# impromptuRong/hd_yolo

Hardware: NVIDIA B200
Metric: postproc_tiles_per_s (higher is better)
Workload: dtype f32

## Files before the change

hd_yolo_b200/csrc/merge.cu:

```cuda
#include "hdy_common.cuh"

namespace hdy {

enum : uint8_t { MS_UNKNOWN = 0, MS_KEPT = 1, MS_SUPPRESSED = 2, MS_DROPPED = 3, MS_REMOTE_UNKNOWN = 4 };

constexpr int kMergeThreads = 256;
constexpr int kMaxRounds = 64;
constexpr float kMergeCellMargin = 1.01f;
constexpr float kMergeMaxScaled = 1.0e6f;

constexpr int kExtBins = 128;
struct MergeStats {
  float ext_sum;
  unsigned ext_cnt;
  float cell_size;
  unsigned ext_hist[kExtBins];
  int unknown[kMaxRounds + 1];
  int rounds_run;
};

constexpr int kScanThreads = 1024;
constexpr int kScanItems = 4;
constexpr int kScanTile = kScanThreads * kScanItems;

__device__ __forceinline__ int block_scan_1024(int v, int* warp_tmp, int& total) {
  const int lane = threadIdx.x & 31, warp = threadIdx.x >> 5;
  int incl = v;
#pragma unroll
  for (int o = 1; o < 32; o <<= 1) {
    int u = __shfl_up_sync(0xffffffffu, incl, o);
    if (lane >= o) incl += u;
  }
  if (lane == 31) warp_tmp[warp] = incl;
  __syncthreads();
  if (warp == 0) {
    int s = warp_tmp[lane], t = s;
#pragma unroll
    for (int o = 1; o < 32; o <<= 1) {
      int u = __shfl_up_sync(0xffffffffu, t, o);
      if (lane >= o) t += u;
    }
    warp_tmp[lane] = t - s;
    if (lane == 31) warp_tmp[32] = t;
  }
  __syncthreads();
  const int excl = warp_tmp[warp] + incl - v;
  total = warp_tmp[32];
  __syncthreads();
  return excl;
}

__global__ void __launch_bounds__(kScanThreads) scan_reduce_kernel(const int* __restrict__ a, long long n,
                                                                    int* __restrict__ block_sums) {
  __shared__ int warp_tmp[33];
  const long long base = (long long)blockIdx.x * kScanTile + (long long)threadIdx.x * kScanItems;
  int s = 0;
#pragma unroll
  for (int k = 0; k < kScanItems; ++k)
    if (base + k < n) s += a[base + k];
  int total;
  block_scan_1024(s, warp_tmp, total);
  if (threadIdx.x == 0) block_sums[blockIdx.x] = total;
}

__global__ void __launch_bounds__(kScanThreads) scan_sums_kernel(int* __restrict__ block_sums, int nblocks,
                                                                  int* __restrict__ total_out) {
  __shared__ int warp_tmp[33];
  __shared__ int carry;
  if (threadIdx.x == 0) carry = 0;
  __syncthreads();
  for (int b0 = 0; b0 < nblocks; b0 += kScanThreads) {
    const int i = b0 + threadIdx.x;
    const int v = i < nblocks ? block_sums[i] : 0;
    int total;
    const int excl = block_scan_1024(v, warp_tmp, total);
    if (i < nblocks) block_sums[i] = carry + excl;
    __syncthreads();
    if (threadIdx.x == 0) carry += total;
    __syncthreads();
  }
  if (threadIdx.x == 0 && total_out) *total_out = carry;
}

__global__ void __launch_bounds__(kScanThreads) scan_apply_kernel(int* __restrict__ a, long long n,
                                                                   const int* __restrict__ block_sums) {
  __shared__ int warp_tmp[33];
  const long long base = (long long)blockIdx.x * kScanTile + (long long)threadIdx.x * kScanItems;
  int v[kScanItems], s = 0;
#pragma unroll
  for (int k = 0; k < kScanItems; ++k) {
    v[k] = (base + k < n) ? a[base + k] : 0;
    s += v[k];
  }
  int total;
  int run = block_sums[blockIdx.x] + block_scan_1024(s, warp_tmp, total);
#pragma unroll
  for (int k = 0; k < kScanItems; ++k) {
    if (base + k < n) a[base + k] = run;
    run += v[k];
  }
}

static inline size_t scan_scratch_ints(long long n) { return (size_t)((n + kScanTile - 1) / kScanTile) + 1; }

static int device_exclusive_scan(int* a, long long n, int* scratch, int* total_out, cudaStream_t st) {
  if (n <= 0) return HDY_OK;
  const int nblocks = (int)((n + kScanTile - 1) / kScanTile);
  scan_reduce_kernel<<<nblocks, kScanThreads, 0, st>>>(a, n, scratch);
  scan_sums_kernel<<<1, kScanThreads, 0, st>>>(scratch, nblocks, total_out);
  scan_apply_kernel<<<nblocks, kScanThreads, 0, st>>>(a, n, scratch);
  return check_launch("device_exclusive_scan");
}

__global__ void __launch_bounds__(1024) append_offsets_kernel(const int32_t* __restrict__ counts, int bs,
                                                               long long* __restrict__ cursor,
                                                               long long* __restrict__ tile_offsets) {
  __shared__ int warp_tmp[33];
  __shared__ long long carry;
  if (threadIdx.x == 0) carry = *cursor;
  __syncthreads();
  for (int b0 = 0; b0 < bs; b0 += 1024) {
    const int i = b0 + threadIdx.x;
    const int v = i < bs ? max(counts[i], 0) : 0;
    int total;
    const int excl = block_scan_1024(v, warp_tmp, total);
    if (i < bs) tile_offsets[i] = carry + excl;
    __syncthreads();
    if (threadIdx.x == 0) carry += total;
    __syncthreads();
  }
  if (threadIdx.x == 0) {
    tile_offsets[bs] = carry;
    *cursor = carry;
  }
}

__global__ void append_tiles_kernel(const float4* __restrict__ boxes, const float* __restrict__ scores,
                                    const int64_t* __restrict__ labels, const uint8_t* __restrict__ fragile,
                                    const int32_t* __restrict__ counts,
                                    const float4* __restrict__ rois, int max_det, int tile_base, float scale,
                                    const long long* __restrict__ tile_offsets, long long capacity,
                                    float4* __restrict__ out_boxes, float* __restrict__ out_scores,
                                    int64_t* __restrict__ out_labels, int32_t* __restrict__ out_tile,
                                    int32_t* __restrict__ status) {
  const int tile = blockIdx.y;
  const int k = min(max(counts[tile], 0), max_det);
  const long long off = tile_offsets[tile];
  const float4 roi = rois[tile];
  for (int d = blockIdx.x * blockDim.x + threadIdx.x; d < k; d += gridDim.x * blockDim.x) {
    const long long o = off + d;
    if (o >= capacity) {
      atomicOr(status, HDY_STATUS_OVERFLOW);
      continue;
    }
    const size_t s = (size_t)tile * max_det + d;
    float4 b = boxes[s];
    if (scale != 1.0f) {
      b.x = __fmul_rn(b.x, scale);
// ... 492 lines not shown
constexpr int kSelMaxBlocks = 4096;

__global__ void __launch_bounds__(kSelThreads) select_count_kernel(const uint8_t* __restrict__ state,
                                                                   const long long* __restrict__ n_dev,
                                                                   long long n_max, long long chunk,
                                                                   int* __restrict__ block_counts) {
  const long long n = n_dev ? min(*n_dev, n_max) : n_max;
  const long long lo = (long long)blockIdx.x * chunk, hi = min(lo + chunk, n);
  int c = 0;
  for (long long i = lo + threadIdx.x; i < hi; i += kSelThreads) c += state[i] == MS_KEPT;
  __shared__ int part[kSelThreads / 32];
#pragma unroll
  for (int o = 16; o > 0; o >>= 1) c += __shfl_xor_sync(0xffffffffu, c, o);
  if ((threadIdx.x & 31) == 0) part[threadIdx.x >> 5] = c;
  __syncthreads();
  if (threadIdx.x == 0) {
    int t = 0;
    for (int w = 0; w < kSelThreads / 32; ++w) t += part[w];
    block_counts[blockIdx.x] = t;
  }
}

__global__ void __launch_bounds__(1024) select_scan_kernel(int* __restrict__ block_counts, int nblocks,
                                                           int* __restrict__ count_out) {
  __shared__ int warp_tmp[33];
  int v[4], s = 0;
#pragma unroll
  for (int j = 0; j < 4; ++j) {
    const int i = threadIdx.x * 4 + j;
    v[j] = i < nblocks ? block_counts[i] : 0;
    s += v[j];
  }
  int total;
  int excl = block_scan_1024(s, warp_tmp, total);
#pragma unroll
  for (int j = 0; j < 4; ++j) {
    const int i = threadIdx.x * 4 + j;
    if (i < nblocks) block_counts[i] = excl;
    excl += v[j];
  }
  if (threadIdx.x == 0) *count_out = total;
}

__global__ void __launch_bounds__(kSelThreads) select_write_kernel(const uint8_t* __restrict__ state,
                                                                   const float* __restrict__ scores,
                                                                   const long long* __restrict__ n_dev,
                                                                   long long n_max, long long chunk,
                                                                   const int* __restrict__ block_offsets,
                                                                   uint64_t* __restrict__ keys) {
  __shared__ int wcount[kSelThreads / 32];
  const long long n = n_dev ? min(*n_dev, n_max) : n_max;
  const long long lo = (long long)blockIdx.x * chunk, hi = min(lo + chunk, n);
  const int lane = threadIdx.x & 31, warp = threadIdx.x >> 5;
  long long running = block_offsets[blockIdx.x];
  for (long long i0 = lo; i0 < hi; i0 += kSelThreads) {
    const long long i = i0 + threadIdx.x;
    const bool k = i < hi && state[i] == MS_KEPT;
    const unsigned m = __ballot_sync(0xffffffffu, k);
    if (lane == 0) wcount[warp] = __popc(m);
    __syncthreads();
    int before = 0, total = 0;
#pragma unroll
    for (int w = 0; w < kSelThreads / 32; ++w) {
      const int c = wcount[w];
      if (w < warp) before += c;
      total += c;
    }
    if (k) keys[running + before + __popc(m & ((1u << lane) - 1u))] = make_key(scores[i], (uint32_t)i);
    running += total;
    __syncthreads();
  }
}

constexpr int kSortThreads = 256;
constexpr int kSortPerWarp = 1024;
constexpr int kSortWarps = kSortThreads / 32;

__global__ void __launch_bounds__(kSortThreads) sort_hist_kernel(const uint64_t* __restrict__ keys,
                                                                  const int* __restrict__ n_dev, int n_max, int shift,
                                                                  int n_sub, int* __restrict__ hist) {
  __shared__ int h[kSortWarps][256];
  const int n = n_dev ? min(*n_dev, n_max) : n_max;
  const int warp = threadIdx.x >> 5, lane = threadIdx.x & 31;
  const int sub = blockIdx.x * kSortWarps + warp;
  for (int d = lane; d < 256; d += 32) h[warp][d] = 0;
  __syncwarp();
  const long long b = (long long)sub * kSortPerWarp;
  for (int k = lane; k < kSortPerWarp; k += 32)
    if (b + k < n) atomicAdd(&h[warp][(int)((keys[b + k] >> shift) & 255)], 1);
  __syncwarp();
  if (sub < n_sub)
    for (int d = lane; d < 256; d += 32) hist[(size_t)d * n_sub + sub] = h[warp][d];
}

__global__ void __launch_bounds__(kSortThreads) sort_scatter_kernel(const uint64_t* __restrict__ keys,
                                                                     const int* __restrict__ n_dev, int n_max,
                                                                     int shift, int n_sub, const int* __restrict__ hist,
                                                                     uint64_t* __restrict__ out) {
  __shared__ int base[kSortWarps][256];
  const int n = n_dev ? min(*n_dev, n_max) : n_max;
  const int warp = threadIdx.x >> 5, lane = threadIdx.x & 31;
  const int sub = blockIdx.x * kSortWarps + warp;
  if (sub >= n_sub) return;
  for (int d = lane; d < 256; d += 32) base[warp][d] = hist[(size_t)d * n_sub + sub];
  __syncwarp();
  const long long b = (long long)sub * kSortPerWarp;
  for (int k0 = 0; k0 < kSortPerWarp; k0 += 32) {
    const long long i = b + k0 + lane;
    const bool valid = i < n;
    const uint64_t key = valid ? keys[i] : 0;
    const int d = valid ? (int)((key >> shift) & 255) : 256 + lane;
    const unsigned peers = __match_any_sync(0xffffffffu, d);
    const int rank = __popc(peers & ((1u << lane) - 1u));
    int dst = 0;
    if (valid) dst = base[warp][d] + rank;
    __syncwarp();
    if (valid && rank == 0) base[warp][d] += __popc(peers);
    __syncwarp();
    if (valid) out[dst] = key;
  }
}

__global__ void merge_gather_kernel(const uint64_t* __restrict__ keys, const int* __restrict__ count, int max_det,
                                    const float4* __restrict__ boxes, const float* __restrict__ scores,
                                    const int64_t* __restrict__ labels, int64_t* __restrict__ out_idx,
                                    float4* __restrict__ out_boxes, float* __restrict__ out_scores,
                                    int64_t* __restrict__ out_labels, int* __restrict__ out_count) {
  const int k = min(*count, max_det);
  if (blockIdx.x == 0 && threadIdx.x == 0) *out_count = k;
  for (int j = blockIdx.x * blockDim.x + threadIdx.x; j < k; j += gridDim.x * blockDim.x) {
    const uint32_t i = key_index(keys[j]);
    if (out_idx) out_idx[j] = (int64_t)i;
    if (out_boxes) out_boxes[j] = boxes[i];
    if (out_scores) out_scores[j] = scores[i];
    if (out_labels && labels) out_labels[j] = labels[i];
  }
}

static inline unsigned blocks_for(long long n, int threads, int max_blocks = 148 * 16) {
  long long b = (n + threads - 1) / threads;
  if (b < 1) b = 1;
  if (b > max_blocks) b = max_blocks;
  return (unsigned)b;
}

constexpr int kSeamHdr = HDY_SEAM_HDR_WORDS, kSeamFar = HDY_SEAM_FAR_WORDS, kSeamRow = HDY_SEAM_ROW_WORDS;
constexpr int kSeamMaxWorld = HDY_SEAM_MAX_WORLD;
enum { SM_NTOTAL = 0, SM_MARGIN = 2, SM_GBASE = 3, SM_FLAGS = 4, SM_FAR_TOTAL = 5, SM_UNDECIDED = 8, SM_REP_OFF = 16,
       SM_OWN_SEAM = 88 };

__device__ __forceinline__ void atomic_min_float(float* addr, float v) {
  if (v >= 0.f)
    atomicMin(reinterpret_cast<int*>(addr), __float_as_int(v));
  else
    atomicMax(reinterpret_cast<unsigned*>(addr), __float_as_uint(v));
}
__device__ __forceinline__ void atomic_max_float(float* addr, float v) {
  if (v >= 0.f)
    atomicMax(reinterpret_cast<int*>(addr), __float_as_int(v));
  else
    atomicMin(reinterpret_cast<unsigned*>(addr), __float_as_uint(v));
}

__global__ void seam_summary_pack_kernel(long long n_local, const float* __restrict__ margin,
                                         const float4* __restrict__ far_boxes, const int32_t* __restrict__ far_tile,
                                         const int32_t* __restrict__ far_count, int far_list_capacity, int tile_base,
                                         int far_cap, int32_t* __restrict__ block) {
  const int k = blockIdx.x * blockDim.x + threadIdx.x;
  const int nf = far_count ? *far_count : 0;
  if (k == 0) {
    float* f = reinterpret_cast<float*>(block);
    const float big = 3.0e38f;
    f[0] = big, f[1] = big, f[2] = -big, f[3] = -big;
    f[4] = margin ? *margin : 0.f;
    block[5] = nf > far_list_capacity ? far_cap + 1 : nf;
    *reinterpret_cast<long long*>(block + 6) = n_local;
// ... 500 lines not shown
  merge_finish_kernel<<<blocks_for(n_max, 256), 256, 0, (cudaStream_t)stream>>>(
      w.pos, w.cstate, reinterpret_cast<const long long*>(n_dev), n_max, state, status);
  return check_launch("hdy_merge_finish");
}

int hdy_merge_nms(const float* boxes, const float* scores, const int32_t* tile_id, const float* tile_cores,
                  const uint8_t* tile_dirty, const float* margin, const int64_t* n_dev, int64_t n_max, float conf_thres,
                  float iou_thres,
                  int max_rounds, uint8_t* state, int32_t* status, void* workspace, size_t workspace_bytes,
                  hdy_stream_t stream) {
  HDY_REQUIRE(max_rounds >= 1 && max_rounds <= kMaxRounds, "hdy_merge_nms: max_rounds out of range [1,%d]", kMaxRounds);
  MergeIn in;
  in.boxes = reinterpret_cast<const float4*>(boxes);
  in.scores = scores;
  in.rep_gidx = nullptr;
  in.gidx_base_dev = nullptr;
  in.tile_base = 0;
  in.tile_id = tile_id;
  in.tile_cores = reinterpret_cast<const float4*>(tile_cores);
  in.tile_dirty = tile_dirty;
  in.margin = margin;
  in.n_dev = reinterpret_cast<const long long*>(n_dev);
  in.n_max = n_max;
  in.n_local = n_max;
  in.conf = conf_thres;
  in.thr = iou_thres;
  int rc = merge_build_common("hdy_merge_nms", in, tile_cores, state, workspace, workspace_bytes, (cudaStream_t)stream);
  if (rc) return rc;
  rc = hdy_merge_rounds(workspace, n_max, iou_thres, 0, max_rounds, stream);
  if (rc) return rc;
  return hdy_merge_finish(workspace, n_dev, n_max, state, status, stream);
}

size_t hdy_sort_workspace_bytes(int64_t n_max) {
  if (n_max <= 0) return 256;
  const long long n_sub = (n_max + kSortPerWarp - 1) / kSortPerWarp;
  const long long hist = 256 * n_sub;
  return align256((size_t)hist * 4) + align256(scan_scratch_ints(hist) * 4);
}

int hdy_sort_keys_bytes(uint64_t* keys, uint64_t* tmp, const int32_t* n_dev, int64_t n_max, int first_byte,
                        int n_bytes, void* workspace, size_t workspace_bytes, hdy_stream_t stream) {
  HDY_REQUIRE(first_byte >= 0 && n_bytes >= 0 && first_byte + n_bytes <= 8 && (n_bytes & 1) == 0,
              "hdy_sort_keys_bytes: bytes [%d, %d) -- an even number of bytes inside the key", first_byte,
              first_byte + n_bytes);
  HDY_REQUIRE(n_max >= 0 && n_max < (1ll << 31), "hdy_sort_keys_bytes: bad size");
  if (n_max == 0) return HDY_OK;
  HDY_REQUIRE(keys && tmp && workspace && workspace_bytes >= hdy_sort_workspace_bytes(n_max),
              "hdy_sort_keys_bytes: NULL pointer or workspace too small");
  cudaStream_t st = (cudaStream_t)stream;
  const int n_sub = (int)((n_max + kSortPerWarp - 1) / kSortPerWarp);
  const long long hist_n = 256ll * n_sub;
  int* hist = static_cast<int*>(workspace);
  int* scratch = reinterpret_cast<int*>(static_cast<unsigned char*>(workspace) + align256((size_t)hist_n * 4));
  const unsigned blocks = (unsigned)((n_sub + kSortWarps - 1) / kSortWarps);
  uint64_t* src = keys;
  uint64_t* dst = tmp;
  for (int pass = first_byte; pass < first_byte + n_bytes; ++pass) {
    sort_hist_kernel<<<blocks, kSortThreads, 0, st>>>(src, n_dev, (int)n_max, pass * 8, n_sub, hist);
    int rc = device_exclusive_scan(hist, hist_n, scratch, nullptr, st);
    if (rc) return rc;
    sort_scatter_kernel<<<blocks, kSortThreads, 0, st>>>(src, n_dev, (int)n_max, pass * 8, n_sub, hist, dst);
    uint64_t* t = src;
    src = dst;
    dst = t;
  }
  return check_launch("hdy_sort_keys_bytes");
}

int hdy_merge_select_ordered(const uint8_t* state, const float* scores, const int64_t* n_dev, int64_t n_max,
                             uint64_t* keys, int32_t* count, int32_t* block_scratch, hdy_stream_t stream) {
  HDY_REQUIRE(n_max >= 0 && n_max < (1ll << 31) && count && block_scratch, "hdy_merge_select_ordered: bad arguments");
  cudaStream_t st = (cudaStream_t)stream;
  if (n_max == 0) {
    cudaError_t e = cudaMemsetAsync(count, 0, 4, st);
    if (e != cudaSuccess) {
      set_error("hdy_merge_select_ordered: %s", cudaGetErrorString(e));
      return HDY_ERR_CUDA;
    }
    return HDY_OK;
  }
  HDY_REQUIRE(state && scores && keys, "hdy_merge_select_ordered: NULL pointer");
  long long chunk = (n_max + kSelMaxBlocks - 1) / kSelMaxBlocks;
  chunk = ((chunk + kSelThreads - 1) / kSelThreads) * kSelThreads;
  if (chunk < 4 * kSelThreads) chunk = 4 * kSelThreads;
  const int nblocks = (int)((n_max + chunk - 1) / chunk);
  const long long* nd = reinterpret_cast<const long long*>(n_dev);
  select_count_kernel<<<nblocks, kSelThreads, 0, st>>>(state, nd, n_max, chunk, block_scratch);
  select_scan_kernel<<<1, 1024, 0, st>>>(block_scratch, nblocks, count);
  select_write_kernel<<<nblocks, kSelThreads, 0, st>>>(state, scores, nd, n_max, chunk, block_scratch, keys);
  return check_launch("hdy_merge_select_ordered");
}

int hdy_merge_gather(const uint64_t* keys, const int32_t* count, int64_t max_det, const float* boxes,
                     const float* scores, const int64_t* labels, int64_t* out_idx, float* out_boxes,
                     float* out_scores, int64_t* out_labels, int32_t* out_count, hdy_stream_t stream) {
  HDY_REQUIRE(max_det >= 0 && max_det < (1ll << 31) && keys && count && out_count, "hdy_merge_gather: bad arguments");
  HDY_REQUIRE((!out_boxes || boxes) && (!out_scores || scores), "hdy_merge_gather: output without its source");
  HDY_REQUIRE((((uintptr_t)boxes | (uintptr_t)out_boxes) & 15) == 0, "hdy_merge_gather: box arrays must be 16-byte aligned");
  merge_gather_kernel<<<blocks_for(max_det > 0 ? max_det : 1, 256), 256, 0, (cudaStream_t)stream>>>(
      keys, count, (int)max_det, reinterpret_cast<const float4*>(boxes), scores, labels, out_idx,
      reinterpret_cast<float4*>(out_boxes), out_scores, out_labels, out_count);
  return check_launch("hdy_merge_gather");
}

}
```

hd_yolo_b200/slide.py:

```python
from __future__ import annotations

import ctypes as C
from typing import Dict, List, Optional, Sequence, Tuple

import torch

from . import _lib
from ._lib import HdyError, ptr
from .ops import DetectBatch, _Scratch, _aligned16, _call, _conf_thr_f32, _iou_thr_f32, _need_cuda, _stream

__all__ = ["sliding_window_scanner", "tile_cores", "merge_outputs", "rescale_outputs", "scale_coords", "clip_coords",
           "merge_nms", "ensemble_merge", "Ensemble", "SlideAccumulator", "sort_keys", "kept_digest", "fold_digest",
           "mask_digest",
           "STATE_KEPT", "STATE_SUPPRESSED", "STATE_DROPPED"]

STATE_UNKNOWN, STATE_KEPT, STATE_SUPPRESSED, STATE_DROPPED = 0, 1, 2, 3
AFFINE_UNPAD, AFFINE_SCALE, AFFINE_CLIP, AFFINE_ROUND = 1, 2, 4, 8
_ws = _Scratch()


def _pair(v):
    return (v, v) if isinstance(v, (int, float)) else (v[0], v[1])


# ... 86 lines not shown
    while True:
        _call("hdy_merge_nms", ptr(boxes), ptr(scores), ptr(tile_id) if use_cores else None,
              ptr(cores) if use_cores else None, ptr(dirty) if use_cores else None,
              ptr(margin) if use_cores else None, ptr(n_dev), n,
              _conf_thr_f32(conf_thres), _iou_thr_f32(iou_thres), rounds, ptr(state), ptr(status), ptr(ws), wbytes,
              _stream(), launches=8 + 3 * rounds)
        if not int(status.item()) & _lib.HDY_STATUS_ROUNDS:
            return state
        if rounds >= 64:
            raise HdyError("merge NMS did not converge in 64 rounds")
        rounds, _ = min(64, rounds * 2), status.zero_()


def dirty_tiles(far_boxes: torch.Tensor, far_tile: torch.Tensor, far_count: torch.Tensor,
                rois: torch.Tensor) -> torch.Tensor:
    n_tiles = int(rois.shape[0])
    dirty = torch.empty((max(n_tiles, 1),), dtype=torch.uint8, device=rois.device)
    _call("hdy_merge_dirty_tiles", ptr(far_boxes), ptr(far_tile), ptr(far_count), int(far_boxes.shape[0]),
          ptr(_aligned16(rois.contiguous())), n_tiles, ptr(dirty), _stream())
    return dirty


def sort_keys(keys: torch.Tensor, n_dev: Optional[torch.Tensor] = None, first_byte: int = 0,
              n_bytes: int = 8) -> torch.Tensor:
    if not keys.is_cuda or keys.dtype != torch.int64 or not keys.is_contiguous():
        raise HdyError("keys must be a contiguous CUDA int64 tensor")
    n = keys.numel()
    if n:
        lib = _lib.load()
        wbytes = lib.hdy_sort_workspace_bytes(n)
        ws = _ws.get(keys.device, "sort", wbytes)
        tmp = _ws.get(keys.device, "sort_tmp", n * 8)
        _call("hdy_sort_keys_bytes", ptr(keys), ptr(tmp), ptr(n_dev), n, int(first_byte), int(n_bytes), ptr(ws), wbytes,
              _stream(), launches=int(n_bytes) * 5)
    return keys


def _order_keys(state, scores, n: int, count: torch.Tensor) -> torch.Tensor:
    dev = scores.device
    keys = torch.empty((max(n, 1),), dtype=torch.int64, device=dev)
    if n == 0:
        count.zero_()
        return keys
    blk = _ws.get(dev, "select_blocks", 4096 * 4)
    _call("hdy_merge_select_ordered", ptr(state), ptr(scores), None, n, ptr(keys), ptr(count), ptr(blk), _stream(),
          launches=3)
    sort_keys(keys, n_dev=count, first_byte=4, n_bytes=4)
    return keys


def _gather_ordered(keys, count, k_all: int, max_det: int, boxes, scores, labels):
    dev = boxes.device
    k = min(int(k_all), int(max_det))
    idx = torch.empty((k,), dtype=torch.int64, device=dev)
    ob = torch.empty((k, 4), dtype=torch.float32, device=dev)
    os_ = torch.empty((k,), dtype=torch.float32, device=dev)
    ol = torch.empty((k,), dtype=torch.int64, device=dev) if labels is not None else None
    oc = torch.empty((1,), dtype=torch.int32, device=dev)
    if k:
        _call("hdy_merge_gather", ptr(keys), ptr(count), k, ptr(boxes), ptr(scores), ptr(labels), ptr(idx), ptr(ob),
              ptr(os_), ptr(ol), ptr(oc), _stream())
    return idx, ob, os_, ol


def _kept_in_order(state, boxes, scores, labels, max_det: int, n_dev=None):
    n = boxes.shape[0]
    count = torch.empty((1,), dtype=torch.int32, device=boxes.device)
# ... 268 lines not shown
```

Before: 161,400.

## Replace per-pass histogram/scan/scatter radix sort with onesweep decoupled-lookback sort

Replaces the three-kernel-per-byte LSD radix sort (warp histograms, device-wide exclusive scan, scatter) with one upfront histogram kernel covering all digit passes, followed by a single onesweep kernel per pass. That kernel ranks keys in shared memory and resolves global offsets through a decoupled lookback over tile prefixes. This cuts the kernel launch count and per-pass global histogram traffic for the kept-box ordering sort, at the cost of spin-waiting on lookback flags and reliance on tile-ticket ordering. The gather kernel is also restructured to handle four items per thread and reuses the score stored in the key where it can.

After: 164,300 (median of 6 runs). +1.8%, better.

```diff
diff --git a/hd_yolo_b200/csrc/merge.cu b/hd_yolo_b200/csrc/merge.cu
--- a/hd_yolo_b200/csrc/merge.cu
+++ b/hd_yolo_b200/csrc/merge.cu
@@ -722,68 +722,49 @@
   }
 }
 
-constexpr int kSortThreads = 256;
-constexpr int kSortPerWarp = 1024;
-constexpr int kSortWarps = kSortThreads / 32;
-
-__global__ void __launch_bounds__(kSortThreads) sort_hist_kernel(const uint64_t* __restrict__ keys,
-                                                                  const int* __restrict__ n_dev, int n_max, int shift,
-                                                                  int n_sub, int* __restrict__ hist) {
-  __shared__ int h[kSortWarps][256];
-  const int n = n_dev ? min(*n_dev, n_max) : n_max;
-  const int warp = threadIdx.x >> 5, lane = threadIdx.x & 31;
-  const int sub = blockIdx.x * kSortWarps + warp;
-  for (int d = lane; d < 256; d += 32) h[warp][d] = 0;
-  __syncwarp();
-  const long long b = (long long)sub * kSortPerWarp;
-  for (int k = lane; k < kSortPerWarp; k += 32)
-    if (b + k < n) atomicAdd(&h[warp][(int)((keys[b + k] >> shift) & 255)], 1);
-  __syncwarp();
-  if (sub < n_sub)
-    for (int d = lane; d < 256; d += 32) hist[(size_t)d * n_sub + sub] = h[warp][d];
-}
-
-__global__ void __launch_bounds__(kSortThreads) sort_scatter_kernel(const uint64_t* __restrict__ keys,
-                                                                     const int* __restrict__ n_dev, int n_max,
-                                                                     int shift, int n_sub, const int* __restrict__ hist,
-                                                                     uint64_t* __restrict__ out) {
-  __shared__ int base[kSortWarps][256];
-  const int n = n_dev ? min(*n_dev, n_max) : n_max;
-  const int warp = threadIdx.x >> 5, lane = threadIdx.x & 31;
-  const int sub = blockIdx.x * kSortWarps + warp;
-  if (sub >= n_sub) return;
-  for (int d = lane; d < 256; d += 32) base[warp][d] = hist[(size_t)d * n_sub + sub];
-  __syncwarp();
-  const long long b = (long long)sub * kSortPerWarp;
-  for (int k0 = 0; k0 < kSortPerWarp; k0 += 32) {
-    const long long i = b + k0 + lane;
-    const bool valid = i < n;
-    const uint64_t key = valid ? keys[i] : 0;
-    const int d = valid ? (int)((key >> shift) & 255) : 256 + lane;
-    const unsigned peers = __match_any_sync(0xffffffffu, d);
-    const int rank = __popc(peers & ((1u << lane) - 1u));
-    int dst = 0;
-    if (valid) dst = base[warp][d] + rank;
-    __syncwarp();
-    if (valid && rank == 0) base[warp][d] += __popc(peers);
-    __syncwarp();
-    if (valid) out[dst] = key;
-  }
-}
-
-__global__ void merge_gather_kernel(const uint64_t* __restrict__ keys, const int* __restrict__ count, int max_det,
-                                    const float4* __restrict__ boxes, const float* __restrict__ scores,
-                                    const int64_t* __restrict__ labels, int64_t* __restrict__ out_idx,
-                                    float4* __restrict__ out_boxes, float* __restrict__ out_scores,
-                                    int64_t* __restrict__ out_labels, int* __restrict__ out_count) {
+constexpr int kGatherThreads = 256;
+constexpr int kGatherItems = 4;
+
+__global__ void __launch_bounds__(kGatherThreads) merge_gather_kernel(
+    const uint64_t* __restrict__ keys, const int* __restrict__ count, int max_det, const float4* __restrict__ boxes,
+    const float* __restrict__ scores, const int64_t* __restrict__ labels, int64_t* __restrict__ out_idx,
+    float4* __restrict__ out_boxes, float* __restrict__ out_scores, int64_t* __restrict__ out_labels,
+    int* __restrict__ out_count) {
   const int k = min(*count, max_det);
   if (blockIdx.x == 0 && threadIdx.x == 0) *out_count = k;
-  for (int j = blockIdx.x * blockDim.x + threadIdx.x; j < k; j += gridDim.x * blockDim.x) {
-    const uint32_t i = key_index(keys[j]);
-    if (out_idx) out_idx[j] = (int64_t)i;
-    if (out_boxes) out_boxes[j] = boxes[i];
-    if (out_scores) out_scores[j] = scores[i];
-    if (out_labels && labels) out_labels[j] = labels[i];
+  const bool want_labels = out_labels && labels;
+  const long long step = (long long)gridDim.x * kGatherThreads * kGatherItems;
+  for (long long j0 = (long long)blockIdx.x * kGatherThreads * kGatherItems + threadIdx.x; j0 < k; j0 += step) {
+    uint32_t row[kGatherItems];
+    float sc[kGatherItems];
+#pragma unroll
+    for (int e = 0; e < kGatherItems; ++e) {
+      const long long j = j0 + e * kGatherThreads;
+      const uint64_t key = j < k ? keys[j] : 0ull;
+      row[e] = key_index(key);
+      sc[e] = key_score(key);
+    }
+    float4 b[kGatherItems];
+    int64_t l[kGatherItems];
+#pragma unroll
+    for (int e = 0; e < kGatherItems; ++e) {
+      if (j0 + e * kGatherThreads < k) {
+        const uint32_t i = row[e];
+        if (out_boxes) b[e] = boxes[i];
+        if (want_labels) l[e] = labels[i];
+        if (out_scores && sc[e] == 0.0f) sc[e] = scores[i];
+      }
+    }
+#pragma unroll
+    for (int e = 0; e < kGatherItems; ++e) {
+      const long long j = j0 + e * kGatherThreads;
+      if (j < k) {
+        if (out_idx) out_idx[j] = (int64_t)row[e];
+        if (out_boxes) out_boxes[j] = b[e];
+        if (out_scores) out_scores[j] = sc[e];
+        if (want_labels) out_labels[j] = l[e];
+      }
+    }
   }
 }
 
@@ -1358,42 +1339,6 @@
   return hdy_merge_finish(workspace, n_dev, n_max, state, status, stream);
 }
 
-size_t hdy_sort_workspace_bytes(int64_t n_max) {
-  if (n_max <= 0) return 256;
-  const long long n_sub = (n_max + kSortPerWarp - 1) / kSortPerWarp;
-  const long long hist = 256 * n_sub;
-  return align256((size_t)hist * 4) + align256(scan_scratch_ints(hist) * 4);
-}
-
-int hdy_sort_keys_bytes(uint64_t* keys, uint64_t* tmp, const int32_t* n_dev, int64_t n_max, int first_byte,
-                        int n_bytes, void* workspace, size_t workspace_bytes, hdy_stream_t stream) {
-  HDY_REQUIRE(first_byte >= 0 && n_bytes >= 0 && first_byte + n_bytes <= 8 && (n_bytes & 1) == 0,
-              "hdy_sort_keys_bytes: bytes [%d, %d) -- an even number of bytes inside the key", first_byte,
-              first_byte + n_bytes);
-  HDY_REQUIRE(n_max >= 0 && n_max < (1ll << 31), "hdy_sort_keys_bytes: bad size");
-  if (n_max == 0) return HDY_OK;
-  HDY_REQUIRE(keys && tmp && workspace && workspace_bytes >= hdy_sort_workspace_bytes(n_max),
-              "hdy_sort_keys_bytes: NULL pointer or workspace too small");
-  cudaStream_t st = (cudaStream_t)stream;
-  const int n_sub = (int)((n_max + kSortPerWarp - 1) / kSortPerWarp);
-  const long long hist_n = 256ll * n_sub;
-  int* hist = static_cast<int*>(workspace);
-  int* scratch = reinterpret_cast<int*>(static_cast<unsigned char*>(workspace) + align256((size_t)hist_n * 4));
-  const unsigned blocks = (unsigned)((n_sub + kSortWarps - 1) / kSortWarps);
-  uint64_t* src = keys;
-  uint64_t* dst = tmp;
-  for (int pass = first_byte; pass < first_byte + n_bytes; ++pass) {
-    sort_hist_kernel<<<blocks, kSortThreads, 0, st>>>(src, n_dev, (int)n_max, pass * 8, n_sub, hist);
-    int rc = device_exclusive_scan(hist, hist_n, scratch, nullptr, st);
-    if (rc) return rc;
-    sort_scatter_kernel<<<blocks, kSortThreads, 0, st>>>(src, n_dev, (int)n_max, pass * 8, n_sub, hist, dst);
-    uint64_t* t = src;
-    src = dst;
-    dst = t;
-  }
-  return check_launch("hdy_sort_keys_bytes");
-}
-
 int hdy_merge_select_ordered(const uint8_t* state, const float* scores, const int64_t* n_dev, int64_t n_max,
                              uint64_t* keys, int32_t* count, int32_t* block_scratch, hdy_stream_t stream) {
   HDY_REQUIRE(n_max >= 0 && n_max < (1ll << 31) && count && block_scratch, "hdy_merge_select_ordered: bad arguments");
@@ -1424,7 +1369,8 @@
   HDY_REQUIRE(max_det >= 0 && max_det < (1ll << 31) && keys && count && out_count, "hdy_merge_gather: bad arguments");
   HDY_REQUIRE((!out_boxes || boxes) && (!out_scores || scores), "hdy_merge_gather: output without its source");
   HDY_REQUIRE((((uintptr_t)boxes | (uintptr_t)out_boxes) & 15) == 0, "hdy_merge_gather: box arrays must be 16-byte aligned");
-  merge_gather_kernel<<<blocks_for(max_det > 0 ? max_det : 1, 256), 256, 0, (cudaStream_t)stream>>>(
+  merge_gather_kernel<<<blocks_for(max_det > 0 ? max_det : 1, kGatherThreads * kGatherItems), kGatherThreads, 0,
+                        (cudaStream_t)stream>>>(
       keys, count, (int)max_det, reinterpret_cast<const float4*>(boxes), scores, labels, out_idx,
       reinterpret_cast<float4*>(out_boxes), out_scores, out_labels, out_count);
   return check_launch("hdy_merge_gather");
diff --git a/hd_yolo_b200/csrc/sort.cu b/hd_yolo_b200/csrc/sort.cu
--- /dev/null
+++ b/hd_yolo_b200/csrc/sort.cu
@@ -0,0 +1,257 @@
+#include "hdy_common.cuh"
+
+namespace hdy {
+
+constexpr int kSortThreads = 256;
+constexpr int kSortWarps = kSortThreads / 32;
+constexpr int kSortItems = 16;
+constexpr int kWarpKeys = kSortItems * 32;
+constexpr int kTile = kSortThreads * kSortItems;
+constexpr int kMaxDigits = 8;
+constexpr int kLookback = 16;
+
+constexpr int kHistItems = 8;
+constexpr int kHistMaxBlocks = 148 * 8;
+
+static inline size_t align256(size_t v) { return (v + 255) & ~(size_t)255; }
+
+constexpr size_t kHeadBytes = 256 * kMaxDigits * 4 + 256;
+
+__device__ __forceinline__ unsigned lanemask_lt() {
+  unsigned m;
+  asm("mov.u32 %0, %%lanemask_lt;" : "=r"(m));
+  return m;
+}
+
+__device__ __forceinline__ unsigned long long ld_relaxed(const unsigned long long* p) {
+  unsigned long long v;
+  asm volatile("ld.relaxed.gpu.global.u64 %0, [%1];" : "=l"(v) : "l"(p) : "memory");
+  return v;
+}
+
+__device__ __forceinline__ void st_relaxed(unsigned long long* p, unsigned long long v) {
+  asm volatile("st.relaxed.gpu.global.u64 [%0], %1;" ::"l"(p), "l"(v) : "memory");
+}
+
+__device__ __forceinline__ unsigned digit_peers(int d, bool valid) {
+  unsigned peers = __ballot_sync(0xffffffffu, valid);
+#pragma unroll
+  for (int bit = 0; bit < 8; ++bit) {
+    const unsigned m = __ballot_sync(0xffffffffu, (d >> bit) & 1);
+    peers &= ((d >> bit) & 1) ? m : ~m;
+  }
+  return peers;
+}
+
+__device__ __forceinline__ int block_scan_256(int v, int* tmp) {
+  const int lane = threadIdx.x & 31, warp = threadIdx.x >> 5;
+  int incl = v;
+#pragma unroll
+  for (int o = 1; o < 32; o <<= 1) {
+    const int u = __shfl_up_sync(0xffffffffu, incl, o);
+    if (lane >= o) incl += u;
+  }
+  if (lane == 31) tmp[warp] = incl;
+  __syncthreads();
+  int before = 0;
+#pragma unroll
+  for (int w = 0; w < kSortWarps; ++w) before += w < warp ? tmp[w] : 0;
+  __syncthreads();
+  return before + incl - v;
+}
+
+__global__ void __launch_bounds__(kSortThreads) sort_hist_kernel(const uint64_t* __restrict__ keys,
+                                                                  const int* __restrict__ n_dev, int n_max,
+                                                                  int first_byte, int n_digits,
+                                                                  unsigned* __restrict__ hist) {
+  __shared__ unsigned h[kMaxDigits * 256];
+  for (int i = threadIdx.x; i < n_digits * 256; i += kSortThreads) h[i] = 0;
+  __syncthreads();
+  const int n = n_dev ? min(*n_dev, n_max) : n_max;
+  const int lane = threadIdx.x & 31, warp = threadIdx.x >> 5;
+  const long long step = (long long)gridDim.x * kSortThreads * kHistItems;
+  for (long long b = ((long long)blockIdx.x * kSortWarps + warp) * 32 * kHistItems; b < n; b += step) {
+    uint64_t k[kHistItems];
+#pragma unroll
+    for (int e = 0; e < kHistItems; ++e) {
+      const long long i = b + e * 32 + lane;
+      k[e] = i < n ? keys[i] : 0ull;
+    }
+    for (int p = 0; p < n_digits; ++p) {
+      const int shift = 8 * (first_byte + p);
+      unsigned* hp = h + p * 256;
+#pragma unroll
+      for (int e = 0; e < kHistItems; ++e) {
+        const bool valid = b + e * 32 + lane < n;
+        const int d = (int)((k[e] >> shift) & 255ull);
+        const int d0 = __shfl_sync(0xffffffffu, d, 0);
+        if (__all_sync(0xffffffffu, valid && d == d0)) {
+          if (lane == 0) atomicAdd(&hp[d0], 32u);
+        } else if (valid) {
+          atomicAdd(&hp[d], 1u);
+        }
+      }
+    }
+  }
+  __syncthreads();
+  for (int i = threadIdx.x; i < n_digits * 256; i += kSortThreads)
+    if (h[i]) atomicAdd(&hist[i], h[i]);
+}
+
+__global__ void __launch_bounds__(kSortThreads) sort_onesweep_kernel(const uint64_t* __restrict__ in,
+                                                                      uint64_t* __restrict__ out,
+                                                                      const int* __restrict__ n_dev, int n_max,
+                                                                      int shift, int pass,
+                                                                      const unsigned* __restrict__ hist,
+                                                                      unsigned* __restrict__ ticket,
+                                                                      unsigned long long* __restrict__ lookback) {
+  __shared__ uint64_t skeys[kTile];
+  __shared__ int whist[kSortWarps][256];
+  __shared__ int gbase[256];
+  __shared__ int tmp[kSortWarps];
+  __shared__ int tile_s;
+  const int t = threadIdx.x, lane = t & 31, warp = t >> 5;
+  if (t == 0) tile_s = (int)atomicAdd(ticket, 1u);
+#pragma unroll
+  for (int w = 0; w < kSortWarps; ++w) whist[w][t] = 0;
+  __syncthreads();
+  const int tile = tile_s;
+  const int n = n_dev ? min(*n_dev, n_max) : n_max;
+  const long long tile_base = (long long)tile * kTile;
+  if (tile_base >= n) return;
+  const int n_tile = (int)min((long long)kTile, n - tile_base);
+
+  uint64_t k[kSortItems];
+  const long long wbase = tile_base + warp * kWarpKeys;
+#pragma unroll
+  for (int e = 0; e < kSortItems; ++e) {
+    const long long i = wbase + e * 32 + lane;
+    k[e] = i < n ? in[i] : 0ull;
+  }
+  const int digit_start = block_scan_256((int)hist[pass * 256 + t], tmp);
+
+  const unsigned lt = lanemask_lt();
+  int loc[kSortItems];
+  int* wh = whist[warp];
+#pragma unroll
+  for (int e = 0; e < kSortItems; ++e) {
+    const bool valid = wbase + e * 32 + lane < n;
+    const int d = (int)((k[e] >> shift) & 255ull);
+    const unsigned peers = digit_peers(d, valid);
+    const int pre = valid ? wh[d] : 0;
+    __syncwarp();
+    if (valid && (peers & lt) == 0) wh[d] = pre + __popc(peers);
+    __syncwarp();
+    loc[e] = pre + __popc(peers & lt);
+  }
+  __syncthreads();
+
+  int count = 0;
+#pragma unroll
+  for (int w = 0; w < kSortWarps; ++w) {
+    const int c = whist[w][t];
+    whist[w][t] = count;
+    count += c;
+  }
+  unsigned long long* my = lookback + (size_t)tile * 256 + t;
+  const unsigned long long tag_own = (unsigned long long)(2 * pass + 1) << 32;
+  const unsigned long long tag_incl = (unsigned long long)(2 * pass + 2) << 32;
+  st_relaxed(my, (tile == 0 ? tag_incl : tag_own) | (unsigned)count);
+  const int local_start = block_scan_256(count, tmp);
+  gbase[t] = local_start;
+  __syncthreads();
+
+#pragma unroll
+  for (int e = 0; e < kSortItems; ++e) {
+    if (wbase + e * 32 + lane < n) {
+      const int d = (int)((k[e] >> shift) & 255ull);
+      skeys[gbase[d] + wh[d] + loc[e]] = k[e];
+    }
+  }
+
+  int before = 0;
+  if (tile > 0) {
+    for (long long j = tile - 1;;) {
+      unsigned long long s[kLookback];
+#pragma unroll
+      for (int q = 0; q < kLookback; ++q) s[q] = j - q >= 0 ? ld_relaxed(lookback + (size_t)(j - q) * 256 + t) : tag_incl;
+      bool done = false;
+      int used = 0;
+#pragma unroll
+      for (int q = 0; q < kLookback; ++q) {
+        const unsigned long long tag = s[q] & 0xffffffff00000000ull;
+        if (tag < tag_own) break;
+        before += (int)(unsigned)s[q];
+        ++used;
+        if (tag == tag_incl) {
+          done = true;
+          break;
+        }
+      }
+      if (done) break;
+      j -= used;
+    }
+    st_relaxed(my, tag_incl | (unsigned)(before + count));
+  }
+  __syncthreads();
+  gbase[t] = digit_start + before - local_start;
+  __syncthreads();
+
+#pragma unroll
+  for (int e = 0; e < kSortItems; ++e) {
+    const int p = e * kSortThreads + t;
+    if (p < n_tile) {
+      const uint64_t key = skeys[p];
+      out[gbase[(int)((key >> shift) & 255ull)] + p] = key;
+    }
+  }
+}
+
+}
+
+using namespace hdy;
+
+extern "C" {
+
+size_t hdy_sort_workspace_bytes(int64_t n_max) {
+  if (n_max <= 0) return 256;
+  const long long n_tiles = (n_max + kTile - 1) / kTile;
+  return kHeadBytes + align256((size_t)n_tiles * 256 * 8);
+}
+
+int hdy_sort_keys_bytes(uint64_t* keys, uint64_t* tmp, const int32_t* n_dev, int64_t n_max, int first_byte,
+                        int n_bytes, void* workspace, size_t workspace_bytes, hdy_stream_t stream) {
+  HDY_REQUIRE(first_byte >= 0 && n_bytes >= 0 && first_byte + n_bytes <= 8 && (n_bytes & 1) == 0,
+              "hdy_sort_keys_bytes: bytes [%d, %d) -- an even number of bytes inside the key", first_byte,
+              first_byte + n_bytes);
+  HDY_REQUIRE(n_max >= 0 && n_max < (1ll << 31), "hdy_sort_keys_bytes: bad size");
+  if (n_max == 0 || n_bytes == 0) return HDY_OK;
+  HDY_REQUIRE(keys && tmp && workspace && workspace_bytes >= hdy_sort_workspace_bytes(n_max),
+              "hdy_sort_keys_bytes: NULL pointer or workspace too small");
+  cudaStream_t st = (cudaStream_t)stream;
+  const long long n_tiles = (n_max + kTile - 1) / kTile;
+  unsigned char* ws = static_cast<unsigned char*>(workspace);
+  unsigned* hist = reinterpret_cast<unsigned*>(ws);
+  unsigned* tickets = hist + 256 * kMaxDigits;
+  unsigned long long* lookback = reinterpret_cast<unsigned long long*>(ws + kHeadBytes);
+  cudaError_t e = cudaMemsetAsync(ws, 0, kHeadBytes + (size_t)n_tiles * 256 * 8, st);
+  if (e != cudaSuccess) {
+    set_error("hdy_sort_keys_bytes: %s", cudaGetErrorString(e));
+    return HDY_ERR_CUDA;
+  }
+  long long hb = (n_max + kSortThreads * kHistItems - 1) / (kSortThreads * kHistItems);
+  if (hb > kHistMaxBlocks) hb = kHistMaxBlocks;
+  sort_hist_kernel<<<(unsigned)hb, kSortThreads, 0, st>>>(keys, n_dev, (int)n_max, first_byte, n_bytes, hist);
+  uint64_t* src = keys;
+  uint64_t* dst = tmp;
+  for (int p = 0; p < n_bytes; ++p) {
+    sort_onesweep_kernel<<<(unsigned)n_tiles, kSortThreads, 0, st>>>(src, dst, n_dev, (int)n_max, 8 * (first_byte + p),
+                                                                     p, hist, tickets + p, lookback);
+    uint64_t* t = src;
+    src = dst;
+    dst = t;
+  }
+  return check_launch("hdy_sort_keys_bytes");
+}
+
+}
diff --git a/hd_yolo_b200/slide.py b/hd_yolo_b200/slide.py
--- a/hd_yolo_b200/slide.py
+++ b/hd_yolo_b200/slide.py
@@ -142,7 +142,7 @@
         ws = _ws.get(keys.device, "sort", wbytes)
         tmp = _ws.get(keys.device, "sort_tmp", n * 8)
         _call("hdy_sort_keys_bytes", ptr(keys), ptr(tmp), ptr(n_dev), n, int(first_byte), int(n_bytes), ptr(ws), wbytes,
-              _stream(), launches=int(n_bytes) * 5)
+              _stream(), launches=int(n_bytes) + 2)
     return keys
 
 
```

## Replace per-pass radix sort with onesweep decoupled-lookback sort and batch gather

Applied to the files above, without the earlier changes.

The radix sort moves from a per-byte histogram, global scan and scatter (five launches per pass) to a single upsweep that builds histograms for all passes at once. Each pass is then one onesweep kernel that ranks keys with warp ballots, stages them in shared memory and gets its global offsets through decoupled lookback across tiles. The gather kernel now handles several rows per thread, reads the score from the key when it is available, and launches at most one resident wave of blocks. This removes many launches and the large per-warp histogram traffic, but the lookback spin relies on tiles being scheduled in ticket order, and occupancy is now queried on every call.

Result: faster. 160,900 before, 164,300 after, median of 6 (+2.1%).

```diff
diff --git a/hd_yolo_b200/csrc/merge.cu b/hd_yolo_b200/csrc/merge.cu
--- a/hd_yolo_b200/csrc/merge.cu
+++ b/hd_yolo_b200/csrc/merge.cu
@@ -23,7 +23,7 @@
 constexpr int kScanItems = 4;
 constexpr int kScanTile = kScanThreads * kScanItems;
 
-__device__ __forceinline__ int block_scan_1024(int v, int* warp_tmp, int& total) {
+__device__ __forceinline__ int block_scan(int v, int* warp_tmp, int& total) {
   const int lane = threadIdx.x & 31, warp = threadIdx.x >> 5;
   int incl = v;
 #pragma unroll
@@ -34,7 +34,7 @@
   if (lane == 31) warp_tmp[warp] = incl;
   __syncthreads();
   if (warp == 0) {
-    int s = warp_tmp[lane], t = s;
+    int s = lane < (int)(blockDim.x >> 5) ? warp_tmp[lane] : 0, t = s;
 #pragma unroll
     for (int o = 1; o < 32; o <<= 1) {
       int u = __shfl_up_sync(0xffffffffu, t, o);
@@ -59,7 +59,7 @@
   for (int k = 0; k < kScanItems; ++k)
     if (base + k < n) s += a[base + k];
   int total;
-  block_scan_1024(s, warp_tmp, total);
+  block_scan(s, warp_tmp, total);
   if (threadIdx.x == 0) block_sums[blockIdx.x] = total;
 }
 
@@ -73,7 +73,7 @@
     const int i = b0 + threadIdx.x;
     const int v = i < nblocks ? block_sums[i] : 0;
     int total;
-    const int excl = block_scan_1024(v, warp_tmp, total);
+    const int excl = block_scan(v, warp_tmp, total);
     if (i < nblocks) block_sums[i] = carry + excl;
     __syncthreads();
     if (threadIdx.x == 0) carry += total;
@@ -93,7 +93,7 @@
     s += v[k];
   }
   int total;
-  int run = block_sums[blockIdx.x] + block_scan_1024(s, warp_tmp, total);
+  int run = block_sums[blockIdx.x] + block_scan(s, warp_tmp, total);
 #pragma unroll
   for (int k = 0; k < kScanItems; ++k) {
     if (base + k < n) a[base + k] = run;
@@ -123,7 +123,7 @@
     const int i = b0 + threadIdx.x;
     const int v = i < bs ? max(counts[i], 0) : 0;
     int total;
-    const int excl = block_scan_1024(v, warp_tmp, total);
+    const int excl = block_scan(v, warp_tmp, total);
     if (i < bs) tile_offsets[i] = carry + excl;
     __syncthreads();
     if (threadIdx.x == 0) carry += total;
@@ -682,7 +682,7 @@
     s += v[j];
   }
   int total;
-  int excl = block_scan_1024(s, warp_tmp, total);
+  int excl = block_scan(s, warp_tmp, total);
 #pragma unroll
   for (int j = 0; j < 4; ++j) {
     const int i = threadIdx.x * 4 + j;
@@ -723,67 +723,199 @@
 }
 
 constexpr int kSortThreads = 256;
-constexpr int kSortPerWarp = 1024;
 constexpr int kSortWarps = kSortThreads / 32;
-
-__global__ void __launch_bounds__(kSortThreads) sort_hist_kernel(const uint64_t* __restrict__ keys,
-                                                                  const int* __restrict__ n_dev, int n_max, int shift,
-                                                                  int n_sub, int* __restrict__ hist) {
-  __shared__ int h[kSortWarps][256];
+constexpr int kSortItems = 16;
+constexpr int kSortWarpKeys = 32 * kSortItems;
+constexpr int kSortTile = kSortThreads * kSortItems;
+constexpr int kSortMaxPasses = 8;
+constexpr int kSortHistCopies = 4;
+constexpr uint32_t kLookInclusive = 1u << 31;
+
+__device__ __forceinline__ uint32_t ld_relaxed_u32(const uint32_t* p) {
+  uint32_t v;
+  asm volatile("ld.relaxed.gpu.global.u32 %0, [%1];" : "=r"(v) : "l"(p) : "memory");
+  return v;
+}
+__device__ __forceinline__ void st_relaxed_u32(uint32_t* p, uint32_t v) {
+  asm volatile("st.relaxed.gpu.global.u32 [%0], %1;" ::"l"(p), "r"(v) : "memory");
+}
+
+__global__ void __launch_bounds__(kSortThreads) sort_upsweep_kernel(const uint64_t* __restrict__ keys,
+                                                                     const int* __restrict__ n_dev, int n_max,
+                                                                     int first_byte, int n_bytes,
+                                                                     uint32_t* __restrict__ hist) {
+  __shared__ uint32_t h[kSortMaxPasses * 256 * kSortHistCopies];
   const int n = n_dev ? min(*n_dev, n_max) : n_max;
-  const int warp = threadIdx.x >> 5, lane = threadIdx.x & 31;
-  const int sub = blockIdx.x * kSortWarps + warp;
-  for (int d = lane; d < 256; d += 32) h[warp][d] = 0;
-  __syncwarp();
-  const long long b = (long long)sub * kSortPerWarp;
-  for (int k = lane; k < kSortPerWarp; k += 32)
-    if (b + k < n) atomicAdd(&h[warp][(int)((keys[b + k] >> shift) & 255)], 1);
-  __syncwarp();
-  if (sub < n_sub)
-    for (int d = lane; d < 256; d += 32) hist[(size_t)d * n_sub + sub] = h[warp][d];
-}
-
-__global__ void __launch_bounds__(kSortThreads) sort_scatter_kernel(const uint64_t* __restrict__ keys,
-                                                                     const int* __restrict__ n_dev, int n_max,
-                                                                     int shift, int n_sub, const int* __restrict__ hist,
-                                                                     uint64_t* __restrict__ out) {
-  __shared__ int base[kSortWarps][256];
+  const int n_tiles = (int)(((long long)n + kSortTile - 1) / kSortTile);
+  const int copy = threadIdx.x & (kSortHistCopies - 1);
+  const int bins = n_bytes * 256;
+  for (int i = threadIdx.x; i < bins * kSortHistCopies; i += kSortThreads) h[i] = 0u;
+  __syncthreads();
+  for (int t = blockIdx.x; t < n_tiles; t += gridDim.x) {
+    const long long base = (long long)t * kSortTile + threadIdx.x;
+    uint64_t k[kSortItems];
+#pragma unroll
+    for (int j = 0; j < kSortItems; ++j) k[j] = base + j * kSortThreads < n ? keys[base + j * kSortThreads] : 0;
+#pragma unroll
+    for (int j = 0; j < kSortItems; ++j) {
+      if (base + j * kSortThreads >= n) break;
+      for (int b = 0; b < n_bytes; ++b)
+        atomicAdd(&h[((b << 8) + (int)((k[j] >> ((first_byte + b) * 8)) & 255)) * kSortHistCopies + copy], 1u);
+    }
+  }
+  __syncthreads();
+  for (int i = threadIdx.x; i < bins; i += kSortThreads) {
+    uint32_t c = 0;
+#pragma unroll
+    for (int k = 0; k < kSortHistCopies; ++k) c += h[i * kSortHistCopies + k];
+    if (c) atomicAdd(&hist[i], c);
+  }
+}
+
+__global__ void __launch_bounds__(256) sort_bases_kernel(uint32_t* __restrict__ hist) {
+  __shared__ int warp_tmp[33];
+  uint32_t* h = hist + blockIdx.x * 256;
+  int sum;
+  h[threadIdx.x] = (uint32_t)block_scan((int)h[threadIdx.x], warp_tmp, sum);
+}
+
+__global__ void __launch_bounds__(kSortThreads, 3) sort_onesweep_kernel(const uint64_t* __restrict__ src,
+                                                                      uint64_t* __restrict__ dst,
+                                                                      const int* __restrict__ n_dev, int n_max,
+                                                                      int shift, const uint32_t* __restrict__ bases,
+                                                                      uint32_t* __restrict__ ticket,
+                                                                      uint32_t* __restrict__ look) {
+  __shared__ uint64_t stage[kSortTile];
+  __shared__ uint32_t wcount[kSortWarps][256];
+  __shared__ int gofs[256];
+  __shared__ int warp_tmp[33];
+  __shared__ int s_part;
+  const int tid = threadIdx.x, lane = tid & 31, warp = tid >> 5;
+  if (tid == 0) s_part = (int)atomicAdd(ticket, 1u);
+#pragma unroll
+  for (int w = 0; w < kSortWarps; ++w) wcount[w][tid] = 0u;
+  __syncthreads();
+  const int part = s_part;
   const int n = n_dev ? min(*n_dev, n_max) : n_max;
-  const int warp = threadIdx.x >> 5, lane = threadIdx.x & 31;
-  const int sub = blockIdx.x * kSortWarps + warp;
-  if (sub >= n_sub) return;
-  for (int d = lane; d < 256; d += 32) base[warp][d] = hist[(size_t)d * n_sub + sub];
-  __syncwarp();
-  const long long b = (long long)sub * kSortPerWarp;
-  for (int k0 = 0; k0 < kSortPerWarp; k0 += 32) {
-    const long long i = b + k0 + lane;
-    const bool valid = i < n;
-    const uint64_t key = valid ? keys[i] : 0;
-    const int d = valid ? (int)((key >> shift) & 255) : 256 + lane;
-    const unsigned peers = __match_any_sync(0xffffffffu, d);
-    const int rank = __popc(peers & ((1u << lane) - 1u));
-    int dst = 0;
-    if (valid) dst = base[warp][d] + rank;
+  const long long tile0 = (long long)part * kSortTile;
+  if (tile0 >= n) return;
+  const int n_valid = (int)min((long long)kSortTile, n - tile0);
+
+  const int wbase = warp * kSortWarpKeys;
+  uint64_t k[kSortItems];
+#pragma unroll
+  for (int j = 0; j < kSortItems; ++j) {
+    const int i = wbase + j * 32 + lane;
+    k[j] = i < n_valid ? src[tile0 + i] : 0;
+  }
+  uint32_t rank[kSortItems];
+  const unsigned lt = (1u << lane) - 1u;
+#pragma unroll
+  for (int j = 0; j < kSortItems; ++j) {
+    const bool valid = wbase + j * 32 + lane < n_valid;
+    const int d = (int)((k[j] >> shift) & 255);
+    unsigned peers = __ballot_sync(0xffffffffu, valid);
+#pragma unroll
+    for (int b = 0; b < 8; ++b) {
+      const unsigned m = __ballot_sync(0xffffffffu, (d >> b) & 1);
+      peers &= ((d >> b) & 1) ? m : ~m;
+    }
+    const uint32_t c = wcount[warp][d];
     __syncwarp();
-    if (valid && rank == 0) base[warp][d] += __popc(peers);
+    const uint32_t below = __popc(peers & lt);
+    if (valid && lane == 31 - __clz(peers)) wcount[warp][d] = c + below + 1u;
     __syncwarp();
-    if (valid) out[dst] = key;
-  }
-}
-
-__global__ void merge_gather_kernel(const uint64_t* __restrict__ keys, const int* __restrict__ count, int max_det,
-                                    const float4* __restrict__ boxes, const float* __restrict__ scores,
-                                    const int64_t* __restrict__ labels, int64_t* __restrict__ out_idx,
-                                    float4* __restrict__ out_boxes, float* __restrict__ out_scores,
-                                    int64_t* __restrict__ out_labels, int* __restrict__ out_count) {
+    rank[j] = c + below;
+  }
+  __syncthreads();
+
+  const int d = tid;
+  uint32_t count = 0;
+#pragma unroll
+  for (int w = 0; w < kSortWarps; ++w) {
+    const uint32_t c = wcount[w][d];
+    wcount[w][d] = count;
+    count += c;
+  }
+  uint32_t* my_look = look + (size_t)part * 256 + d;
+  st_relaxed_u32(my_look, part == 0 ? kLookInclusive | count : count + 1u);
+  int total;
+  const int lstart = block_scan((int)count, warp_tmp, total);
+  gofs[d] = lstart;
+  __syncthreads();
+#pragma unroll
+  for (int j = 0; j < kSortItems; ++j)
+    if (wbase + j * 32 + lane < n_valid) {
+      const int dj = (int)((k[j] >> shift) & 255);
+      stage[gofs[dj] + (int)wcount[warp][dj] + (int)rank[j]] = k[j];
+    }
+
+  uint32_t excl = 0;
+  if (part > 0) {
+    for (const uint32_t* p = my_look - 256;; p -= 256) {
+      uint32_t v;
+      do {
+        v = ld_relaxed_u32(p);
+      } while (v == 0u);
+      if (v & kLookInclusive) {
+        excl += v & ~kLookInclusive;
+        break;
+      }
+      excl += v - 1u;
+    }
+    st_relaxed_u32(my_look, kLookInclusive | (excl + count));
+  }
+  __syncthreads();
+  gofs[d] = (int)(bases[d] + excl) - lstart;
+  __syncthreads();
+#pragma unroll
+  for (int j = 0; j < kSortItems; ++j) {
+    const int i = j * kSortThreads + tid;
+    if (i < n_valid) {
+      const uint64_t key = stage[i];
+      dst[gofs[(int)((key >> shift) & 255)] + i] = key;
+    }
+  }
+}
+
+constexpr int kGatherThreads = 256;
+constexpr int kGatherRows = 8;
+
+__global__ void __launch_bounds__(kGatherThreads) merge_gather_kernel(
+    const uint64_t* __restrict__ keys, const int* __restrict__ count, int max_det, const float4* __restrict__ boxes,
+    const float* __restrict__ scores, const int64_t* __restrict__ labels, int64_t* __restrict__ out_idx,
+    float4* __restrict__ out_boxes, float* __restrict__ out_scores, int64_t* __restrict__ out_labels,
+    int* __restrict__ out_count) {
   const int k = min(*count, max_det);
   if (blockIdx.x == 0 && threadIdx.x == 0) *out_count = k;
-  for (int j = blockIdx.x * blockDim.x + threadIdx.x; j < k; j += gridDim.x * blockDim.x) {
-    const uint32_t i = key_index(keys[j]);
-    if (out_idx) out_idx[j] = (int64_t)i;
-    if (out_boxes) out_boxes[j] = boxes[i];
-    if (out_scores) out_scores[j] = scores[i];
-    if (out_labels && labels) out_labels[j] = labels[i];
+  const long long step = (long long)gridDim.x * kGatherRows * kGatherThreads;
+  for (long long j0 = (long long)blockIdx.x * kGatherRows * kGatherThreads + threadIdx.x; j0 < k; j0 += step) {
+    uint64_t key[kGatherRows];
+#pragma unroll
+    for (int r = 0; r < kGatherRows; ++r) key[r] = j0 + r * kGatherThreads < k ? keys[j0 + r * kGatherThreads] : 0;
+    float4 b[kGatherRows];
+    float s[kGatherRows];
+    int64_t l[kGatherRows];
+#pragma unroll
+    for (int r = 0; r < kGatherRows; ++r) {
+      if (j0 + r * kGatherThreads >= k) break;
+      const uint32_t i = key_index(key[r]);
+      if (out_boxes) b[r] = boxes[i];
+      if (out_labels && labels) l[r] = labels[i];
+      if (out_scores) {
+        s[r] = key_score(key[r]);
+        if (s[r] == 0.f || s[r] != s[r]) s[r] = scores[i];
+      }
+    }
+#pragma unroll
+    for (int r = 0; r < kGatherRows; ++r) {
+      const long long j = j0 + r * kGatherThreads;
+      if (j >= k) break;
+      if (out_idx) out_idx[j] = (int64_t)key_index(key[r]);
+      if (out_boxes) out_boxes[j] = b[r];
+      if (out_scores) out_scores[j] = s[r];
+      if (out_labels && labels) out_labels[j] = l[r];
+    }
   }
 }
 
@@ -792,6 +924,40 @@
   if (b < 1) b = 1;
   if (b > max_blocks) b = max_blocks;
   return (unsigned)b;
+}
+
+template <typename Kernel>
+static int resident_ctas(Kernel kernel, int threads) {
+  int dev = 0, sms = 0, per_sm = 0;
+  if (cudaGetDevice(&dev) != cudaSuccess ||
+      cudaDeviceGetAttribute(&sms, cudaDevAttrMultiProcessorCount, dev) != cudaSuccess ||
+      cudaOccupancyMaxActiveBlocksPerMultiprocessor(&per_sm, kernel, threads, 0) != cudaSuccess)
+    return 0;
+  return sms * per_sm;
+}
+
+struct SortWs {
+  uint32_t* hist;
+  uint32_t* ticket;
+  uint32_t* look;
+  size_t look_bytes;
+  size_t bytes;
+  int parts;
+};
+
+static SortWs sort_layout(void* base, long long n_max) {
+  SortWs w;
+  w.parts = (int)((n_max + kSortTile - 1) / kSortTile);
+  unsigned char* p = static_cast<unsigned char*>(base);
+  size_t o = 0;
+  w.hist = reinterpret_cast<uint32_t*>(p + o);
+  o += align256((size_t)kSortMaxPasses * 256 * 4);
+  w.ticket = reinterpret_cast<uint32_t*>(p + o);
+  w.look = reinterpret_cast<uint32_t*>(p + o + 256);
+  w.look_bytes = 256 + (size_t)w.parts * 256 * 4;
+  o += align256(w.look_bytes);
+  w.bytes = o;
+  return w;
 }
 
 constexpr int kSeamHdr = HDY_SEAM_HDR_WORDS, kSeamFar = HDY_SEAM_FAR_WORDS, kSeamRow = HDY_SEAM_ROW_WORDS;
@@ -1360,9 +1526,7 @@
 
 size_t hdy_sort_workspace_bytes(int64_t n_max) {
   if (n_max <= 0) return 256;
-  const long long n_sub = (n_max + kSortPerWarp - 1) / kSortPerWarp;
-  const long long hist = 256 * n_sub;
-  return align256((size_t)hist * 4) + align256(scan_scratch_ints(hist) * 4);
+  return sort_layout(nullptr, n_max).bytes;
 }
 
 int hdy_sort_keys_bytes(uint64_t* keys, uint64_t* tmp, const int32_t* n_dev, int64_t n_max, int first_byte,
@@ -1371,22 +1535,35 @@
               "hdy_sort_keys_bytes: bytes [%d, %d) -- an even number of bytes inside the key", first_byte,
               first_byte + n_bytes);
   HDY_REQUIRE(n_max >= 0 && n_max < (1ll << 31), "hdy_sort_keys_bytes: bad size");
-  if (n_max == 0) return HDY_OK;
+  if (n_max == 0 || n_bytes == 0) return HDY_OK;
   HDY_REQUIRE(keys && tmp && workspace && workspace_bytes >= hdy_sort_workspace_bytes(n_max),
               "hdy_sort_keys_bytes: NULL pointer or workspace too small");
   cudaStream_t st = (cudaStream_t)stream;
-  const int n_sub = (int)((n_max + kSortPerWarp - 1) / kSortPerWarp);
-  const long long hist_n = 256ll * n_sub;
-  int* hist = static_cast<int*>(workspace);
-  int* scratch = reinterpret_cast<int*>(static_cast<unsigned char*>(workspace) + align256((size_t)hist_n * 4));
-  const unsigned blocks = (unsigned)((n_sub + kSortWarps - 1) / kSortWarps);
+  const SortWs w = sort_layout(workspace, n_max);
+  const int resident = resident_ctas(sort_upsweep_kernel, kSortThreads);
+  if (resident <= 0) {
+    set_error("hdy_sort_keys_bytes: occupancy query failed");
+    return HDY_ERR_CUDA;
+  }
+  cudaError_t e = cudaMemsetAsync(w.hist, 0, (size_t)n_bytes * 256 * 4, st);
+  if (e != cudaSuccess) {
+    set_error("hdy_sort_keys_bytes: cudaMemsetAsync: %s", cudaGetErrorString(e));
+    return HDY_ERR_CUDA;
+  }
+  sort_upsweep_kernel<<<(unsigned)min(w.parts, resident), kSortThreads, 0, st>>>(keys, n_dev, (int)n_max, first_byte,
+                                                                                 n_bytes, w.hist);
+  sort_bases_kernel<<<n_bytes, 256, 0, st>>>(w.hist);
   uint64_t* src = keys;
   uint64_t* dst = tmp;
-  for (int pass = first_byte; pass < first_byte + n_bytes; ++pass) {
-    sort_hist_kernel<<<blocks, kSortThreads, 0, st>>>(src, n_dev, (int)n_max, pass * 8, n_sub, hist);
-    int rc = device_exclusive_scan(hist, hist_n, scratch, nullptr, st);
-    if (rc) return rc;
-    sort_scatter_kernel<<<blocks, kSortThreads, 0, st>>>(src, n_dev, (int)n_max, pass * 8, n_sub, hist, dst);
+  for (int b = 0; b < n_bytes; ++b) {
+    e = cudaMemsetAsync(w.ticket, 0, w.look_bytes, st);
+    if (e != cudaSuccess) {
+      set_error("hdy_sort_keys_bytes: cudaMemsetAsync: %s", cudaGetErrorString(e));
+      return HDY_ERR_CUDA;
+    }
+    sort_onesweep_kernel<<<(unsigned)w.parts, kSortThreads, 0, st>>>(src, dst, n_dev, (int)n_max, (first_byte + b) * 8,
+                                                                      w.hist + b * 256, w.ticket,
+                                                                      w.look);
     uint64_t* t = src;
     src = dst;
     dst = t;
@@ -1424,7 +1601,13 @@
   HDY_REQUIRE(max_det >= 0 && max_det < (1ll << 31) && keys && count && out_count, "hdy_merge_gather: bad arguments");
   HDY_REQUIRE((!out_boxes || boxes) && (!out_scores || scores), "hdy_merge_gather: output without its source");
   HDY_REQUIRE((((uintptr_t)boxes | (uintptr_t)out_boxes) & 15) == 0, "hdy_merge_gather: box arrays must be 16-byte aligned");
-  merge_gather_kernel<<<blocks_for(max_det > 0 ? max_det : 1, 256), 256, 0, (cudaStream_t)stream>>>(
+  const int resident = resident_ctas(merge_gather_kernel, kGatherThreads);
+  if (resident <= 0) {
+    set_error("hdy_merge_gather: occupancy query failed");
+    return HDY_ERR_CUDA;
+  }
+  const long long chunks = (max_det + kGatherRows * kGatherThreads - 1) / (kGatherRows * kGatherThreads);
+  merge_gather_kernel<<<(unsigned)max(1ll, min(chunks, (long long)resident)), kGatherThreads, 0, (cudaStream_t)stream>>>(
       keys, count, (int)max_det, reinterpret_cast<const float4*>(boxes), scores, labels, out_idx,
       reinterpret_cast<float4*>(out_boxes), out_scores, out_labels, out_count);
   return check_launch("hdy_merge_gather");
diff --git a/hd_yolo_b200/slide.py b/hd_yolo_b200/slide.py
--- a/hd_yolo_b200/slide.py
+++ b/hd_yolo_b200/slide.py
@@ -142,7 +142,7 @@
         ws = _ws.get(keys.device, "sort", wbytes)
         tmp = _ws.get(keys.device, "sort_tmp", n * 8)
         _call("hdy_sort_keys_bytes", ptr(keys), ptr(tmp), ptr(n_dev), n, int(first_byte), int(n_bytes), ptr(ws), wbytes,
-              _stream(), launches=int(n_bytes) * 5)
+              _stream(), launches=int(n_bytes) + 2)
     return keys
 
 
```
